# Banus/pano360

Hardware: AMD Instinct MI355X
Metric: blended megapixels/sec (multiband) (higher is better)
Workload: dtype f32; 1 GPU; cfg3: 32 synthetic 3840x2160 frames per image set, spherical warp + multiband blend L=5, native resolution (MAX_RESOLUTION uncapped); frames=32

## Files before the change

### include/pano360.h

```cpp
#ifndef PANO360_H
#define PANO360_H

#include <stddef.h>
#include <stdint.h>

#ifdef __cplusplus
extern "C" {
#endif

#define PANO_OK 0
#define PANO_EINVAL (-1)
#define PANO_EHIP (-2)
#define PANO_ELIMIT (-3)
#define PANO_ESOLVE (-4)

#define PANO_MAX_TAPS 129
#define PANO_MAX_LEVELS 8
#define PANO_TAP_LEAD 7
#define PANO_TAP_PAD 40
#ifndef PANO_INTERIOR_BLOCK
#define PANO_INTERIOR_BLOCK 4
#endif

typedef struct pano_patch {
// ... 38 lines not shown
    float angle;
    float response;
    int32_t octave;
    int32_t r, c;
} pano_sift_keypoint;


const char *pano_version(void);
const char *pano_last_error(void);
int pano_device_count(void);
int pano_pitch(int w);
int pano_interior_block(void);

typedef struct pano_ctx pano_ctx;
#define PANO_OPT_BLUR_KERNEL 0
#define PANO_OPT_OWN_PRUNE 1
#define PANO_OPT_BLUR_SEGMENTS 2
#define PANO_OPT_BLUR_LEAN 3
#define PANO_OPT_STITCH_STREAMS 4
#define PANO_OPT_STITCH_ASYNC 5
#define PANO_OPT_BLUR_SEG_LEN 6
#define PANO_OPT_SIFT_GRAPH 7
#define PANO_OPT_LEVEL_CLASSES 8
#define PANO_OPT_COUNT 9
#define PANO_BLUR_MFMA 0
#define PANO_BLUR_VALU 1
int pano_ctx_create(int device, void *stream, pano_ctx **out);
int pano_ctx_destroy(pano_ctx *ctx);
int pano_ctx_set_stream(pano_ctx *ctx, void *stream);
int pano_ctx_set_option(pano_ctx *ctx, int option, int value);
int pano_ctx_get_option(const pano_ctx *ctx, int option, int *value);

int pano_timing_enable(pano_ctx *ctx, int on);
int pano_kernel_count(void);
const char *pano_kernel_name(int kid);
int pano_timing_read(pano_ctx *ctx, int kid, double *total_ms, int *launches);

int pano_add_weights(pano_ctx *ctx, const uint8_t *frame, int h, int w,
                     const float *lut255, const double *hat_x, const double *hat_y,
                     float *rgba);

int pano_warp_spherical(pano_ctx *ctx, const uint8_t *frame, int sh, int sw,
                        const double *proj, const double *sin_t, const double *cos_t,
                        const double *tan_p, const float *lut255, const double *hat_x,
                        const double *hat_y, int gx0, int gy0, int pw, int ph,
                        float *planes, uint8_t *mask, float *map_x, float *map_y);

// ... 257 lines not shown
```

### pano360_amd/_lib.py

```python
import ctypes as C
import os
import subprocess

_HERE = os.path.dirname(os.path.abspath(__file__))
LIB_PATH = os.environ.get("PANO_LIB") or os.path.join(_HERE, "libpano360_hip.so")

MAX_TAPS = 129
MAX_LEVELS = 8
TAP_LEAD = 7
TAP_PAD = 40
OPT_BLUR_KERNEL, OPT_OWN_PRUNE, OPT_BLUR_SEGMENTS, OPT_BLUR_LEAN, OPT_STITCH_STREAMS = 0, 1, 2, 3, 4
OPT_STITCH_ASYNC = 5
OPT_BLUR_SEG_LEN = 6
OPT_SIFT_GRAPH = 7
OPT_LEVEL_CLASSES = 8
BLUR_MFMA, BLUR_VALU = 0, 1


class PanoError(RuntimeError):
    """A C-ABI call returned a negative status."""


class Patch(C.Structure):
    _fields_ = [("planes", C.c_void_p), ("mask", C.c_void_p),
                ("blurred", C.c_void_p), ("scratch", C.c_void_p),
                ("y0", C.c_int32), ("x0", C.c_int32), ("h", C.c_int32), ("w", C.c_int32),
                ("vy0", C.c_int32), ("vx0", C.c_int32), ("vh", C.c_int32), ("vw", C.c_int32),
                ("ay0", C.c_int32), ("ax0", C.c_int32), ("ah", C.c_int32), ("aw", C.c_int32),
                ("vpitch", C.c_int32), ("apitch", C.c_int32),
                ("index", C.c_int32), ("tiles_off", C.c_int32)]


class Layout(C.Structure):
    _fields_ = [("planes_floats", C.c_int64), ("blurred_floats", C.c_int64),
                ("scratch_floats", C.c_int64), ("n_records", C.c_int32), ("n_tiles", C.c_int32),
                ("max_vw", C.c_int32), ("max_vh", C.c_int32), ("max_aw", C.c_int32),
                ("max_ah", C.c_int32), ("missing", C.c_int32)]

# ... 205 lines not shown
```

### pano360_amd/csrc/api.hip

```cpp
#include <stdarg.h>
#include <stdio.h>
#include <stdlib.h>
#include <string.h>

#include <vector>

#include "common.h"
#include "layout.h"

static thread_local char g_error[512] = "";

void pano_set_error(const char *fmt, ...) {
    va_list ap;
    va_start(ap, fmt);
    vsnprintf(g_error, sizeof(g_error), fmt, ap);
    va_end(ap);
}

extern "C" const char *pano_version(void) { return "pano360_hip 0.1 (gfx950)"; }

extern "C" const char *pano_last_error(void) { return g_error; }

extern "C" int pano_device_count(void) {
    int n = 0;
// ... 8 lines not shown

extern "C" int pano_interior_block(void) { return PANO_INTERIOR_BLOCK; }

extern "C" int pano_ctx_create(int device, void *stream, pano_ctx **out) {
    PANO_REQUIRE(out, "pano_ctx_create: null output");
    *out = nullptr;
    PANO_REQUIRE(device >= 0 && device < pano_device_count(), "pano_ctx_create: no device %d",
                 device);
    PANO_HIP(hipSetDevice(device));
    if (int rc = pano_blur_mfma_opt_in()) return rc;
    if (int rc = pano_blur_valu_opt_in()) return rc;
    pano_ctx *ctx = new pano_ctx();
    ctx->device = device;
    ctx->stream = (hipStream_t)stream;
    ctx->opt[PANO_OPT_BLUR_KERNEL] = PANO_BLUR_MFMA;
    ctx->opt[PANO_OPT_OWN_PRUNE] = 1;
    ctx->opt[PANO_OPT_BLUR_SEGMENTS] = 1;
    ctx->opt[PANO_OPT_BLUR_LEAN] = 1;
    ctx->opt[PANO_OPT_STITCH_STREAMS] = 1;
    ctx->opt[PANO_OPT_STITCH_ASYNC] = 0;
    ctx->opt[PANO_OPT_BLUR_SEG_LEN] = 0;
    ctx->opt[PANO_OPT_SIFT_GRAPH] = 1;
    ctx->opt[PANO_OPT_LEVEL_CLASSES] = 0;
    *out = ctx;
    return PANO_OK;
}

int pano_ctx_enter(pano_ctx *ctx) {
    if (!ctx->in_stitch) ctx->geom_valid = false;
    PANO_HIP(hipSetDevice(ctx->device));
    return PANO_OK;
}

static void timing_clear(pano_ctx *ctx) {
    for (int k = 0; k < PK_COUNT; ++k) {
        for (hipEvent_t e : ctx->t_begin[k]) (void)hipEventDestroy(e);
        for (hipEvent_t e : ctx->t_end[k]) (void)hipEventDestroy(e);
        ctx->t_begin[k].clear();
        ctx->t_end[k].clear();
    }
}

static void tap_set_free(PanoTapSet &ts) {
    if (ts.taps) (void)hipFree(ts.taps);
    if (ts.tables) (void)hipFree(ts.tables);
    if (ts.ready) (void)hipEventDestroy(ts.ready);
// ... 151 lines not shown
    return PANO_OK;
}

int pano_ctx_tap_set_built(pano_ctx *ctx, PanoTapSet *set) {
    PANO_HIP(hipEventRecord(set->ready, ctx->stream));
    set->built_on = ctx->stream;
    return PANO_OK;
}

static const char *const g_kernel_names[] = {
    "add_weights_kernel", "warp_spherical_kernel", "ownership_kernel", "blur_rows_kernel",
    "blur_cols_kernel",   "multiband_compose_kernel", "linear_blend_kernel",
    "no_blend_kernel",    "crop_heights_kernel", "crop_rows_kernel", "pyr_down_kernel",
    "ownership_cameras_kernel", "owned_boxes_kernel", "warp_windows_kernel",
    "blend_cameras_kernel", "owned_spans_kernel",
    "block_owner_kernel", "tile_flags_kernel", "overlap_stats_kernel",
    "blur_mfma_kernel", "sift_extrema_kernel", "sift_orient_kernel", "sift_describe_kernel",
    "scale_step_kernel", "knn2_kernel", "blur_lean_kernel", "blur_lean5_kernel",
    "ransac_score_kernel", "ransac_finish_kernel", "match_pack_kernel",
    "ba_residual_kernel", "ba_pair_kernel", "ba_assemble_kernel",
    "jpeg_destuff_kernel", "jpeg_scan_kernel", "jpeg_intervals_kernel", "jpeg_huff_sync_kernel",
    "jpeg_huff_write_kernel", "jpeg_dc_kernel", "jpeg_idct_kernel", "jpeg_pixels_kernel",
    "jpeg_enc_blocks_kernel", "jpeg_enc_count_kernel", "jpeg_enc_scan_kernel", "jpeg_enc_emit_kernel",
    "jpeg_enc_stuff_kernel"};
static_assert(sizeof(g_kernel_names) / sizeof(g_kernel_names[0]) == PK_COUNT,
              "one name per PanoKernelId, in enum order");

void pano_timing_edge(pano_ctx *ctx, int kid, hipStream_t stream, bool begin) {
    hipEvent_t ev;
    if (hipEventCreate(&ev) != hipSuccess) return;
    (void)hipEventRecord(ev, stream);
    (begin ? ctx->t_begin : ctx->t_end)[kid].push_back(ev);
}

extern "C" int pano_timing_enable(pano_ctx *ctx, int on) {
    PANO_REQUIRE(ctx, "pano_timing_enable: null context");
    timing_clear(ctx);
    ctx->timing_on = on != 0;
    return PANO_OK;
}

extern "C" int pano_kernel_count(void) { return PK_COUNT; }

extern "C" const char *pano_kernel_name(int kid) {
    return kid >= 0 && kid < PK_COUNT ? g_kernel_names[kid] : "";
}

// ... 83 lines not shown
```

### pano360_amd/csrc/blend.hip

```cpp
#include <stdlib.h>

#include "geom.h"

__global__ __launch_bounds__(256) void ownership_kernel(
    const pano_patch *__restrict__ patches, int n, int H, int W,
    int16_t *__restrict__ owner, uint8_t *__restrict__ valid) {
    const int x = blockIdx.x * 64 + threadIdx.x, y = blockIdx.y * 4 + threadIdx.y;
    if (x >= W || y >= H) return;
    float best = 0.0f;
    int who = -1;
    bool any = false;
    for (int i = 0; i < n; ++i) {
        const pano_patch p = patches[i];
        const int px = x - p.x0, py = y - p.y0;
        if ((unsigned)px >= (unsigned)p.w || (unsigned)py >= (unsigned)p.h) continue;
        const float a = p.planes[3 * (size_t)p.vh * p.vpitch + (size_t)py * p.vpitch + px];
        if (a > best) {
            best = a;
            who = i;
        }
        any |= p.mask[(size_t)py * p.w + px] == 0;
    }
    owner[(size_t)y * W + x] = (int16_t)who;
    valid[(size_t)y * W + x] = any ? 1 : 0;
// ... 643 lines not shown
enum { LUT_LDS = 0, LUT_GLOBAL = 1 };

template <int LUT>
__device__ __forceinline__ void shade_interior(const pano_camera *cam, const float *__restrict__ table,
                                               const InteriorArgs &ia, int x, int y, int W,
                                               uint8_t *__restrict__ mosaic,
                                               float *__restrict__ mosaic_f32) {
    if (!cam->frame) return;
    const int sw = cam->sw, sh = cam->sh;
    float fx, fy;
    map_pixel(cam->proj, table_f64(ia.sin_t, x), table_f64(ia.cos_t, x), table_f64(ia.tan_p, y), sw, sh, fx, fy);
    Taps tp = tap_base(fx, fy);
    TapBytes tb;
    if (__ballot(!taps_interior(tp, sw, sh)) == 0ull) {
        tb = load_taps_interior(cam->frame, sw, tp);
    } else {
        tp.x1 = min(tp.x1, sw - 1);
        tp.y1 = min(tp.y1, sh - 1);
        tb = load_taps(cam->frame, sw, tp);
    }
    const size_t g = ((size_t)y * W + x) * 3;
#pragma unroll
    for (int c = 0; c < 3; ++c) {
        float v = lerp4(lut_at(table, tb.v[0][c]), lut_at(table, tb.v[1][c]),
                        lut_at(table, tb.v[2][c]), lut_at(table, tb.v[3][c]), tp);
        v = v < 0.0f ? 0.0f : (v > 1.0f ? 1.0f : v);
        if (mosaic_f32) mosaic_f32[g + c] = v;
        mosaic[g + c] = (uint8_t)(int)(255.0f * v);
    }
}

template <int LUT>
__device__ __forceinline__ void shade_interior_of(int own, const float *__restrict__ table, int stride,
                                                  const InteriorArgs &ia, int x, int y, int W,
                                                  uint8_t *__restrict__ mosaic,
                                                  float *__restrict__ mosaic_f32) {
    const int own_u = __builtin_amdgcn_readfirstlane(own);
    if (__ballot(own != own_u) == 0)
        shade_interior<LUT>(ia.cams + own_u, table + (size_t)own_u * stride, ia, x, y, W, mosaic, mosaic_f32);
    else
        shade_interior<LUT>(ia.cams + own, table + (size_t)own * stride, ia, x, y, W, mosaic, mosaic_f32);
}

#define COMPOSE_MASKS 4
template <int L, bool PERCAM, bool CLS>
__global__ __launch_bounds__(256) void multiband_compose_kernel(
    const pano_patch *__restrict__ patches, int n, int H, int W, int xs0, int xs1,
    const int16_t *__restrict__ owner, const uint8_t *__restrict__ valid,
    uint8_t *__restrict__ mosaic, float *__restrict__ mosaic_f32, InteriorArgs ia) {
    __shared__ float s_lut[256];
    if (ia.interior && !PERCAM) {
        s_lut[threadIdx.y * 64 + threadIdx.x] = ia.lut[threadIdx.y * 64 + threadIdx.x];
        __syncthreads();
    }
    const int x = xs0 + blockIdx.x * 64 + threadIdx.x, y = blockIdx.y * 4 + threadIdx.y;
    const bool inside = x < xs1 && y < H;
    const bool is_interior = inside && ia.interior && ia.interior[(size_t)(y / IB) * ia.W8 + x / IB];
    unsigned long long cand[COMPOSE_MASKS] = {};
    const bool masked = n <= 64 * COMPOSE_MASKS && __ballot(inside && !is_interior) != 0;
    if (masked) {
        const int wx0 = xs0 + blockIdx.x * 64, wx1 = min(wx0 + 64, xs1);
#pragma unroll
        for (int m = 0; m < COMPOSE_MASKS; ++m) {
            const int i = 64 * m + (int)threadIdx.x;
            bool hit = false;
            if (i < n) {
                const pano_patch *q = patches + i;
                const int ax = q->x0 + q->ax0, ay = q->y0 + q->ay0;
                hit = ax < wx1 && ax + q->aw > wx0 && ay <= y && y < ay + q->ah;
            }
            cand[m] = __ballot(hit);
        }
    }
    if (!inside) return;
    if (is_interior) {
        const int own = owner[(size_t)y * W + x];
        if (PERCAM)
            shade_interior_of<LUT_GLOBAL>(own, ia.lut, 256, ia, x, y, W, mosaic, mosaic_f32);
        else
            shade_interior_of<LUT_LDS>(own, s_lut, 0, ia, x, y, W, mosaic, mosaic_f32);
        return;
    }
    float layer[L][3], wsum[L];
#pragma unroll
    for (int k = 0; k < L; ++k) layer[k][0] = layer[k][1] = layer[k][2] = wsum[k] = 0.0f;
    const int j = CLS && L > 1 ? (int)ia.classes[(size_t)(y / IB) * ia.W8 + x / IB] : 0;
    const int own_px = CLS && j > 0 ? (int)owner[(size_t)y * W + x] : -1;
    float base[3] = {0.0f, 0.0f, 0.0f};

    int m = 0;
    unsigned long long bits = masked ? cand[0] : 0ull;
    for (int i = 0;; ++i) {
        if (masked) {
            while (bits == 0ull && ++m < COMPOSE_MASKS) bits = cand[m];
            if (bits == 0ull) break;
            i = 64 * m + __ffsll((long long)bits) - 1;
            bits &= bits - 1ull;
        } else if (i >= n) {
// ... 353 lines not shown
extern "C" int pano_interior_map(pano_ctx *ctx, const int16_t *owner, int H, int W, int xs0,
                                 int xs1, int radius, int16_t *block_owner, uint8_t *interior) {
    PANO_ENTER(ctx, "pano_interior_map");
    return interior_map_launch(ctx, owner, H, W, xs0, xs1, &radius, 1, block_owner, interior, nullptr,
                               "pano_interior_map");
}

extern "C" int pano_interior_classes(pano_ctx *ctx, const int16_t *owner, int H, int W, int xs0,
                                     int xs1, const int *radii, int n_radii, int16_t *block_owner,
                                     uint8_t *interior, uint8_t *classes) {
    PANO_ENTER(ctx, "pano_interior_classes");
    PANO_REQUIRE(classes, "pano_interior_classes: null pointer");
    return interior_map_launch(ctx, owner, H, W, xs0, xs1, radii, n_radii, block_owner, interior,
                               classes, "pano_interior_classes");
}

extern "C" int pano_multiband_compose(pano_ctx *ctx, const pano_patch *patches, int n, int H,
                                      int W, int xs0, int xs1, int n_levels, const int16_t *owner,
                                      const uint8_t *valid, const uint8_t *interior,
                                      const uint8_t *classes, const pano_camera *cams,
                                      const double *sin_t,
                                      const double *cos_t, const double *tan_p, const float *lut,
                                      int lut_stride, uint8_t *mosaic, float *mosaic_f32) {
    PANO_ENTER(ctx, "pano_multiband_compose");
    if (int rc = check_table(patches, n, H, W, "pano_multiband_compose")) return rc;
    PANO_REQUIRE(H > 0 && W > 0, "pano_multiband_compose: bad mosaic shape %dx%d", H, W);
    PANO_REQUIRE(owner && mosaic && valid, "pano_multiband_compose: null pointer");
    PANO_REQUIRE(n_levels >= 1 && n_levels <= PANO_MAX_LEVELS,
                 "pano_multiband_compose: n_levels %d outside [1, %d]", n_levels, PANO_MAX_LEVELS);
    PANO_REQUIRE(xs0 >= 0 && xs1 <= W && xs0 <= xs1,
                 "pano_multiband_compose: bad strip [%d, %d)", xs0, xs1);
    PANO_REQUIRE(!interior || (cams && sin_t && cos_t && tan_p && lut),
                 "pano_multiband_compose: the interior map needs cameras, tables and LUT");
    PANO_REQUIRE(lut_stride == 0 || lut_stride == 256,
                 "pano_multiband_compose: lut_stride %d (0 = shared table, 256 = per camera)",
                 lut_stride);
    if (xs0 == xs1) return PANO_OK;
    PANO_REQUIRE(!classes || interior, "pano_multiband_compose: level classes without the interior map");
    InteriorArgs ia = {interior, ceil_div(W, IB), cams, sin_t, cos_t, tan_p, lut,
                       ctx->opt[PANO_OPT_LEVEL_CLASSES] ? classes : nullptr};
    const bool percam = interior && lut_stride != 0;
    dim3 block(64, 4), grid(ceil_div(xs1 - xs0, 64), ceil_div(H, 4));
    hipStream_t s = (hipStream_t)stream;
#define COMPOSE_AS(L, PC, CL)                                                            \
    PANO_TIMED(PK_COMPOSE, s,                                                           \
               hipLaunchKernelGGL((multiband_compose_kernel<L, PC, CL>), grid, block, 0, s, \
                                  patches, n, H, W, xs0, xs1, owner, valid, mosaic,     \
                                  mosaic_f32, ia))
#define COMPOSE(L)                                                                      \
    case L:                                                                             \
        if (ia.classes && L > 1) {                                                      \
            if (percam) COMPOSE_AS(L, true, true); else COMPOSE_AS(L, false, true);     \
        } else {                                                                        \
            if (percam) COMPOSE_AS(L, true, false); else COMPOSE_AS(L, false, false);   \
        }                                                                               \
        break;
    switch (n_levels) {
        COMPOSE(1) COMPOSE(2) COMPOSE(3) COMPOSE(4) COMPOSE(5) COMPOSE(6) COMPOSE(7) COMPOSE(8)
    }
#undef COMPOSE_AS
#undef COMPOSE
    PANO_LAUNCH_CHECK("multiband_compose_kernel");
    return PANO_OK;
}

extern "C" int pano_linear_blend(pano_ctx *ctx, const pano_patch *patches, int n, int H, int W,
                                 uint8_t *mosaic) {
    PANO_ENTER(ctx, "pano_linear_blend");
    if (int rc = check_table(patches, n, H, W, "pano_linear_blend")) return rc;
    PANO_REQUIRE(mosaic, "pano_linear_blend: null output");
    MOSAIC_GRID;
    PANO_TIMED(PK_LINEAR, (hipStream_t)stream,
               hipLaunchKernelGGL(linear_blend_kernel, grid, block, 0, (hipStream_t)stream,
                                  patches, n, H, W, mosaic));
    PANO_LAUNCH_CHECK("linear_blend_kernel");
    return PANO_OK;
}

extern "C" int pano_no_blend(pano_ctx *ctx, const pano_patch *patches, int n, int H, int W,
                             uint8_t *mosaic) {
    PANO_ENTER(ctx, "pano_no_blend");
    if (int rc = check_table(patches, n, H, W, "pano_no_blend")) return rc;
    PANO_REQUIRE(mosaic, "pano_no_blend: null output");
// ... 8 lines not shown
```

### pano360_amd/csrc/common.h

```cpp
#pragma once
#include <hip/hip_runtime.h>
#include <stdint.h>

#include <vector>

#include "../../include/pano360.h"

void pano_set_error(const char *fmt, ...);

#define PANO_REQUIRE(cond, ...)          \
    do {                                 \
        if (!(cond)) {                   \
            pano_set_error(__VA_ARGS__); \
            return PANO_EINVAL;          \
        }                                \
    } while (0)

#define PANO_HIP(call)                                                         \
    do {                                                                       \
        hipError_t e_ = (call);                                                \
        if (e_ != hipSuccess) {                                                \
            pano_set_error("%s failed: %s", #call, hipGetErrorString(e_));     \
            return PANO_EHIP;                                                  \
        }                                                                      \
// ... 36 lines not shown
    PK_SCALE_STEP,
    PK_KNN2,
    PK_BLUR_LEAN,
    PK_BLUR_LEAN5,
    PK_RANSAC_SCORE,
    PK_RANSAC_FINISH,
    PK_MATCH_PACK,
    PK_BA_RESIDUAL,
    PK_BA_PAIRS,
    PK_BA_ASSEMBLE,
    PK_JPEG_DESTUFF,
    PK_JPEG_SCAN,
    PK_JPEG_INTERVALS,
    PK_JPEG_HUFF_SYNC,
    PK_JPEG_HUFF_WRITE,
    PK_JPEG_DC,
    PK_JPEG_IDCT,
    PK_JPEG_PIXELS,
    PK_JPEG_ENC_BLOCKS,
    PK_JPEG_ENC_COUNT,
    PK_JPEG_ENC_SCAN,
    PK_JPEG_ENC_EMIT,
    PK_JPEG_ENC_STUFF,
    PK_COUNT
};
struct PanoTapSet {
    uint64_t key;
    int n, ntaps[PANO_MAX_LEVELS];
    float *taps;
    unsigned char *tables;
    uint64_t used;
    float *host;
    size_t floats;
    hipEvent_t ready;
    hipStream_t built_on;
};

struct LayoutSummary;
struct PanoSiftGraph {
    uint64_t key;
    hipGraphExec_t exec;
    int seen;
    uint64_t used;
};

#define GEOM_BUFS 11
// ... 32 lines not shown
    bool geom_valid, in_stitch;
    const void *geom_bufs[GEOM_BUFS];
    int lay_count[2];
    uint32_t *sift_raw;
    size_t sift_raw_cap;
    bool sift_capturing;
    std::vector<PanoSiftGraph> sift_graphs;
    uint8_t *enc_dev, *enc_out, *enc_host;
    size_t enc_dev_cap, enc_out_cap, enc_host_cap;
    uint8_t *poisson_dev, *poisson_host;
    size_t poisson_cap;
    uint8_t *seam_dev, *seam_host;
};

int pano_ctx_enter(pano_ctx *ctx);
void pano_sift_graphs_free(pano_ctx *ctx);
int pano_sift_raw_reserve(pano_ctx *ctx, int rows, int cols);
int pano_zero_i32(hipStream_t s, int *p, int n);
int pano_ctx_side_stream(pano_ctx *ctx);
int pano_ctx_tap_set(pano_ctx *ctx, const float *taps, const int *ntaps, int n, size_t table_bytes,
                     PanoTapSet **out, bool *fresh);
int pano_ctx_tap_set_built(pano_ctx *ctx, PanoTapSet *set);

#define PANO_ENTER(ctx, who)                                       \
    PANO_REQUIRE((ctx) != nullptr, "%s: null context", who);       \
    if (int rc_ = pano_ctx_enter(ctx)) return rc_;                 \
    void *const stream = (void *)(ctx)->stream;                    \
    (void)stream

#define PANO_ENTER_READONLY(ctx, who)                              \
    const bool geom_keep_ = (ctx) != nullptr && (ctx)->geom_valid; \
    PANO_ENTER(ctx, who);                                          \
    (ctx)->geom_valid = geom_keep_

void pano_timing_edge(pano_ctx *ctx, int kid, hipStream_t stream, bool begin);

#define PANO_TIMED(kid, stream, ...)                                        \
    do {                                                                    \
        if (ctx->timing_on) pano_timing_edge(ctx, kid, stream, true);       \
        __VA_ARGS__;                                                        \
        if (ctx->timing_on) pano_timing_edge(ctx, kid, stream, false);      \
    } while (0)

static inline int pano_pitch_of(int w) { return (w + 3) & ~3; }

int pano_launch_blur_mfma(pano_ctx *ctx, const pano_patch *table, int n, int max_aw, int max_ah,
// ... 42 lines not shown
```

### pano360_amd/csrc/geom.h

```cpp
#pragma once
#include "common.h"

struct Taps {
    int x0, x1, y0, y1;
    float w00, w01, w10, w11;
};

__device__ __forceinline__ Taps tap_base(float px, float py) {
    int sx = cv_round(px * 32.0f), sy = cv_round(py * 32.0f);
    int fx = sx & 31, fy = sy & 31;
    Taps t;
    t.x0 = sat16(sx >> 5);
    t.y0 = sat16(sy >> 5);
    t.x1 = t.x0 + 1;
    t.y1 = t.y0 + 1;
    float ax = (float)fx * (1.0f / 32.0f), ay = (float)fy * (1.0f / 32.0f);
    t.w00 = (1.0f - ay) * (1.0f - ax);
    t.w01 = (1.0f - ay) * ax;
    t.w10 = ay * (1.0f - ax);
    t.w11 = ay * ax;
    return t;
}

__device__ __forceinline__ void reflect_taps(Taps &t, int sw, int sh) {
// ... 7 lines not shown
    Taps t = tap_base(px, py);
    reflect_taps(t, sw, sh);
    return t;
}

__device__ __forceinline__ bool taps_interior(const Taps &t, int sw, int sh) {
    return (unsigned)t.x0 < (unsigned)(sw - 1) && (unsigned)t.y0 < (unsigned)(sh - 1);
}

__device__ __forceinline__ Taps make_taps_unmasked(float px, float py, int sw, int sh) {
    Taps t = tap_base(px, py);
    t.x1 = min(t.x1, sw - 1);
    t.y1 = min(t.y1, sh - 1);
    return t;
}

__device__ __forceinline__ float lerp4(float v00, float v01, float v10, float v11,
                                       const Taps &t) {
    float a = v00 * t.w00;
    a = a + v01 * t.w01;
    a = a + v10 * t.w10;
    a = a + v11 * t.w11;
    return a;
}

struct TapBytes {
    uint32_t v[4][3];
};
typedef uint32_t u32_any __attribute__((aligned(1)));
typedef uint16_t u16_any __attribute__((aligned(1)));
typedef const __attribute__((address_space(1))) uint8_t *frame_ptr;
typedef const __attribute__((address_space(1))) u32_any *frame_ptr32;
typedef const __attribute__((address_space(1))) u16_any *frame_ptr16;

#define PANO_BYTE_X4(B)                                                                        \
    __device__ __forceinline__ uint32_t byte##B##_x4(uint32_t x) {                             \
        uint32_t r;                                                                            \
        asm("v_lshlrev_b32_sdwa %0, %1, %2 dst_sel:DWORD dst_unused:UNUSED_PAD "               \
            "src0_sel:DWORD src1_sel:BYTE_" #B                                                 \
            : "=v"(r)                                                                          \
            : "v"(2u), "v"(x));                                                                \
        return r;                                                                              \
    }
PANO_BYTE_X4(0)
PANO_BYTE_X4(1)
PANO_BYTE_X4(2)
// ... 84 lines not shown
```

### pano360_amd/csrc/stitch.hip

```cpp
#include <string.h>

#include "common.h"
#include "layout.h"


#define LAY_THREADS 512
__global__ __launch_bounds__(LAY_THREADS) void layout_windows_kernel(
    const int32_t *__restrict__ regions, const int32_t *__restrict__ rects,
    const uint8_t *__restrict__ have, int n, int max_spans, int radius, int xs0, int xs1,
    int n_blur, int grid32, float *planes, float *blurred, float *scratch, long cap_planes,
    long cap_blurred, long cap_scratch, int cap_tiles, int want_tiles, int b_nr, int b_vw,
    int b_vh, int b_aw, int b_ah, pano_patch *__restrict__ table,
    LayoutSummary *__restrict__ summary, LayoutSummary expect, int check_expect,
    int *__restrict__ sticky) {
    __shared__ long s_planes[LAY_THREADS], s_blurred[LAY_THREADS], s_scratch[LAY_THREADS];
    __shared__ int s_tiles[LAY_THREADS], s_slot[LAY_THREADS];
    __shared__ long s_run[4];
    __shared__ int s_count, s_max[4], s_missing, s_bad;
    const int tid = threadIdx.x, stride = 5 + 2 * max_spans;
    if (tid == 0) {
        s_run[0] = s_run[1] = s_run[2] = s_run[3] = 0;
        s_count = s_missing = s_bad = 0;
        s_max[0] = s_max[1] = s_max[2] = s_max[3] = 0;
    }
// ... 204 lines not shown
    }
    a->used_need = 0;
    if (kept) {
        a->used_need = need_choice == 1;
        two_streams = false;
    } else if (interior && tile_grid == 32 && nr && a->tile_flags && a->need) {
        bool on = need_choice == 1;
        if (need_choice < 0) {
            double sum = 0.0;
            for (int k = 0; k < nr; ++k) sum += a->records_host[k].aw;
            on = sum / nr >= 768.0;
        }
        if (on) {
            if (two_streams) {
                PANO_HIP(hipEventRecord(ctx->ev_join, ctx->side));
                PANO_HIP(hipStreamWaitEvent(s, ctx->ev_join, 0));
            }
            if (int rc = pano_blur_tiles(ctx, a->table, nr, lay.max_aw, lay.max_ah, a->W, a->radius,
                                         a->interior, a->tile_flags, a->need))
                return rc;
            a->used_need = 1;
        }
    }
    const bool fork2 = two_streams && interior && n_blur && nr &&
                       !a->used_need && tile_grid == 32 && a->tile_flags;
    if (fork2) {
        if (device_table) {
            PANO_HIP(hipEventRecord(ctx->ev_upload, s));
        }
        PANO_HIP(hipStreamWaitEvent(ctx->side, ctx->ev_upload, 0));
        ON_SIDE(ctx, pano_multiband_blur_prepare(ctx, a->table, nr, lay.max_aw, lay.max_ah, a->W,
                                                 a->interior, a->tile_flags));
        PANO_HIP(hipEventRecord(ctx->ev_join, ctx->side));
    } else if (two_streams && interior) {
        PANO_HIP(hipEventRecord(ctx->ev_join, ctx->side));
    }
    if (int rc = pano_warp_windows(ctx, a->cams, a->table, nr, lay.max_vw, lay.max_vh, a->sin_t,
                                   a->cos_t, a->tan_p, a->lut, a->lut_stride,
                                   a->used_need ? a->need : nullptr))
        return rc;
    if (two_streams && interior) PANO_HIP(hipStreamWaitEvent(s, ctx->ev_join, 0));
    if (kept && use_blur) {
        ctx->prepared_table = a->table;
        ctx->prepared_n = nr;
    }
    if (n_blur)
        if (int rc = pano_multiband_blur(ctx, a->table, nr, lay.max_aw, lay.max_vh, lay.max_ah,
                                         a->owner, a->W, a->taps, (const int *)a->ntaps, n_blur,
                                         interior ? a->interior : nullptr,
                                         interior ? a->tile_flags : nullptr))
            return rc;
    return pano_multiband_compose(ctx, a->table, nr, a->H, a->W, a->xs0, a->xs1, a->n_levels,
                                  a->owner, a->valid, interior ? a->interior : nullptr,
                                  interior && stitch_has_classes(ctx, a, n_blur) ? a->classes : nullptr,
                                  interior ? a->cams : nullptr, interior ? a->sin_t : nullptr,
                                  interior ? a->cos_t : nullptr, interior ? a->tan_p : nullptr,
                                  a->lut, a->lut_stride, a->mosaic, a->mosaic_f32);
}

static void geometry_buffers(const pano_stitch_args *a, const void *out[GEOM_BUFS]) {
    const void *v[GEOM_BUFS] = {a->owner, a->valid, a->table, a->interior, a->tile_flags, a->need,
                                a->planes, a->blurred, a->scratch, a->sin_t, a->classes};
    for (int k = 0; k < GEOM_BUFS; ++k) out[k] = v[k];
}
static void geometry_left(pano_ctx *ctx, const pano_stitch_args *a) {
    geometry_buffers(a, ctx->geom_bufs);
    ctx->geom_valid = true;
}

namespace {
struct StitchScope {
    pano_ctx *ctx;
    explicit StitchScope(pano_ctx *c) : ctx(c) { ctx->in_stitch = true; }
    ~StitchScope() { ctx->in_stitch = false; }
};
}

extern "C" int pano_stitch_multiband(pano_ctx *ctx, pano_stitch_args *a, int resume) {
    const bool geom_was_valid = ctx && ctx->geom_valid;
    PANO_ENTER(ctx, "pano_stitch_multiband");
// ... 225 lines not shown
```

### pano360_amd/csrc/warp.hip

```cpp
#include "geom.h"

struct ProjK {
    double p[9];
};

template <bool FULL>
__global__ __launch_bounds__(256) void warp_spherical_kernel(
    const uint8_t *__restrict__ frame, int sh, int sw, ProjK K,
    const double *__restrict__ sin_t, const double *__restrict__ cos_t,
    const double *__restrict__ tan_p, const float *__restrict__ lut255,
    const double *__restrict__ hat_x, const double *__restrict__ hat_y,
    int gx0, int gy0, int pw, int ph, int pitch, float *__restrict__ planes,
    uint8_t *__restrict__ mask, float *__restrict__ map_x,
    float *__restrict__ map_y) {
    __shared__ float s_lut[256];
    s_lut[threadIdx.y * 64 + threadIdx.x] = lut255[threadIdx.y * 64 + threadIdx.x];
    __syncthreads();

    const int x = blockIdx.x * 64 + threadIdx.x;
    const int y = blockIdx.y * 4 + threadIdx.y;
    if (x >= pw || y >= ph) return;

    float px, py;
    const bool m = map_pixel(K.p, sin_t[gx0 + x], cos_t[gx0 + x], tan_p[gy0 + y], sw, sh,
// ... 2 lines not shown
    const uint8_t *r0 = frame + (size_t)tp.y0 * sw * 3;
    const uint8_t *r1 = frame + (size_t)tp.y1 * sw * 3;
    const uint8_t *p00 = r0 + tp.x0 * 3, *p01 = r0 + tp.x1 * 3;
    const uint8_t *p10 = r1 + tp.x0 * 3, *p11 = r1 + tp.x1 * 3;
    const size_t plane = (size_t)ph * pitch;
    const size_t o = (size_t)y * pitch + x;
#pragma unroll
    for (int k = 0; k < 3; ++k)
        planes[k * plane + o] =
            lerp4(s_lut[p00[k]], s_lut[p01[k]], s_lut[p10[k]], s_lut[p11[k]], tp);
    if (FULL) {
        float a = alpha_at(hat_x, hat_y, tp);
        a = a * (m ? 0.0f : 1.0f);
        planes[3 * plane + o] = a;
        mask[(size_t)y * pw + x] = m ? 1 : 0;
        if (map_x) {
            map_x[(size_t)y * pw + x] = px;
            map_y[(size_t)y * pw + x] = py;
        }
    }
}

#define WARP_ROWS 4
__global__ __launch_bounds__(256) void warp_windows_kernel(
    const pano_camera *__restrict__ cams, const pano_patch *__restrict__ patches,
    const double *__restrict__ sin_t, const double *__restrict__ cos_t,
    const double *__restrict__ tan_p, const float *__restrict__ lut, int lut_stride,
    const uint8_t *__restrict__ need) {
    __shared__ float s_lut[256];
    const pano_patch p = patches[blockIdx.z];
    constexpr int BH = 4 * WARP_ROWS;
    if ((int)blockIdx.x * 64 >= p.vw || (int)blockIdx.y * BH >= p.vh) return;
    if (need) {
        const int ntx = ((p.ax0 + p.aw - 1) >> 5) - (p.ax0 >> 5) + 1;
        const int nty = ((p.ay0 + p.ah - 1) >> 5) - (p.ay0 >> 5) + 1;
        const int px0 = p.vx0 + (int)blockIdx.x * 64, py0 = p.vy0 + (int)blockIdx.y * BH;
        const int ty0 = min(max((py0 >> 5) - (p.ay0 >> 5), 0), nty - 1);
        const int ty1 = min(max(((py0 + BH - 1) >> 5) - (p.ay0 >> 5), 0), nty - 1);
        const int tx0 = min(max((px0 >> 5) - (p.ax0 >> 5), 0), ntx - 1);
        const int tx1 = min(max(((px0 + 63) >> 5) - (p.ax0 >> 5), 0), ntx - 1);
        bool any = false;
        for (int ty = ty0; ty <= ty1; ++ty)
            for (int tx = tx0; tx <= tx1; ++tx) any |= need[p.tiles_off + ty * ntx + tx] != 0;
        if (!any) return;
    }
    s_lut[threadIdx.y * 64 + threadIdx.x] =
        lut[(size_t)p.index * lut_stride + threadIdx.y * 64 + threadIdx.x];
    __syncthreads();

    const int x = blockIdx.x * 64 + threadIdx.x;
    const int y0 = blockIdx.y * BH + threadIdx.y;
    if (x >= p.vw || y0 >= p.vh) return;
    const pano_camera *cam = cams + p.index;
    const int sw = cam->sw, sh = cam->sh;
    const int gx = p.x0 + p.vx0 + x;
    const double s = table_f64(sin_t, gx), c = table_f64(cos_t, gx);
    double t[WARP_ROWS];
#pragma unroll
    for (int j = 0; j < WARP_ROWS; ++j)
        t[j] = table_f64(tan_p, p.y0 + p.vy0 + min(y0 + 4 * j, p.vh - 1));
    Taps tp[WARP_ROWS];
    TapBytes tb[WARP_ROWS];
    bool inner = true;
#pragma unroll
    for (int j = 0; j < WARP_ROWS; ++j) {
        float px, py;
        map_pixel(cam->proj, s, c, t[j], sw, sh, px, py);
        tp[j] = tap_base(px, py);
        inner &= taps_interior(tp[j], sw, sh);
    }
    if (__ballot(!inner) == 0ull) {
#pragma unroll
        for (int j = 0; j < WARP_ROWS; ++j) tb[j] = load_taps_interior(cam->frame, sw, tp[j]);
    } else {
#pragma unroll
        for (int j = 0; j < WARP_ROWS; ++j) {
            reflect_taps(tp[j], sw, sh);
            tb[j] = load_taps(cam->frame, sw, tp[j]);
        }
    }
    typedef __attribute__((address_space(1))) float *plane_ptr;
    typedef __attribute__((address_space(1))) char *byte_ptr;
    const size_t plane = (size_t)p.vh * p.vpitch;
    const byte_ptr out[3] = {(byte_ptr)p.planes, (byte_ptr)(p.planes + plane),
                             (byte_ptr)(p.planes + 2 * plane)};
#pragma unroll
    for (int j = 0; j < WARP_ROWS; ++j) {
        const int y = y0 + 4 * j;
        if (y >= p.vh) break;
        const uint32_t o = ((uint32_t)y * (uint32_t)p.vpitch + (uint32_t)x) * 4u;
#pragma unroll
        for (int k = 0; k < 3; ++k) {
            *(plane_ptr)(out[k] + o) = lerp4(lut_at(s_lut, tb[j].v[0][k]), lut_at(s_lut, tb[j].v[1][k]),
                                             lut_at(s_lut, tb[j].v[2][k]), lut_at(s_lut, tb[j].v[3][k]), tp[j]);
        }
    }
}

__global__ __launch_bounds__(256) void add_weights_kernel(
    const uint8_t *__restrict__ frame, int h, int w,
    const float *__restrict__ lut255, const double *__restrict__ hat_x,
    const double *__restrict__ hat_y, float4 *__restrict__ rgba) {
    const int x = blockIdx.x * 64 + threadIdx.x;
    const int y = blockIdx.y * 4 + threadIdx.y;
    if (x >= w || y >= h) return;
    const uint8_t *s = frame + ((size_t)y * w + x) * 3;
    float4 v;
    v.x = lut255[s[0]];
    v.y = lut255[s[1]];
    v.z = lut255[s[2]];
    v.w = (float)(hat_y[y] * hat_x[x]);
    rgba[(size_t)y * w + x] = v;
}

extern "C" int pano_add_weights(pano_ctx *ctx, const uint8_t *frame, int h, int w,
                                const float *lut255, const double *hat_x, const double *hat_y,
                                float *rgba) {
// ... 31 lines not shown
    for (int i = 0; i < 9; ++i) K.p[i] = proj[i];
    dim3 block(64, 4), grid(ceil_div(pw, 64), ceil_div(ph, 4));
    PANO_TIMED(PK_WARP, (hipStream_t)stream,
               hipLaunchKernelGGL(warp_spherical_kernel<true>, grid, block, 0,
                                  (hipStream_t)stream, frame, sh, sw, K, sin_t, cos_t, tan_p,
                                  lut255, hat_x, hat_y, gx0, gy0, pw, ph, pano_pitch_of(pw),
                                  planes, mask, map_x, map_y));
    PANO_LAUNCH_CHECK("warp_spherical_kernel");
    return PANO_OK;
}

extern "C" int pano_warp_windows(pano_ctx *ctx, const pano_camera *cams, const pano_patch *patches,
                                 int n, int max_vw, int max_vh, const double *sin_t,
                                 const double *cos_t, const double *tan_p, const float *lut,
                                 int lut_stride, const uint8_t *need) {
    PANO_ENTER(ctx, "pano_warp_windows");
    PANO_REQUIRE(cams && patches && sin_t && cos_t && tan_p && lut && lut_stride >= 0,
                 "pano_warp_windows: null pointer");
    PANO_REQUIRE(n >= 0 && n <= 65535 && max_vw >= 0 && max_vh >= 0,
                 "pano_warp_windows: bad argument");
    if (n == 0 || max_vw == 0 || max_vh == 0) return PANO_OK;
    dim3 block(64, 4), grid(ceil_div(max_vw, 64), ceil_div(max_vh, 4 * WARP_ROWS), n);
    PANO_TIMED(PK_WARP_WINDOWS, (hipStream_t)stream,
               hipLaunchKernelGGL(warp_windows_kernel, grid, block, 0, (hipStream_t)stream,
                                  cams, patches, sin_t, cos_t, tan_p, lut, lut_stride, need));
    PANO_LAUNCH_CHECK("warp_windows_kernel");
    return PANO_OK;
}
```

Baseline: 209,900 MP/s.

## Fuse interior mosaic shading into the window warp kernel

When the interior map is available and level classes are off, the window warp kernel also writes the final 8-bit (and optional f32) mosaic pixels for interior blocks owned by the current camera. It packs RGB bytes across the wavefront with shuffles so rows are stored as aligned dwords. The compose kernel then runs an unshaded variant that skips interior pixels, so the separate per-pixel re-projection and bilinear resampling in compose goes away. The cost is extra owner and interior-map reads in warp, masked byte stores, and a new stream join before the warp, which serializes the side stream earlier.

```diff
diff --git a/include/pano360.h b/include/pano360.h
--- a/include/pano360.h
+++ b/include/pano360.h
@@ -84,7 +84,8 @@
 #define PANO_OPT_BLUR_SEG_LEN 6
 #define PANO_OPT_SIFT_GRAPH 7
 #define PANO_OPT_LEVEL_CLASSES 8
-#define PANO_OPT_COUNT 9
+#define PANO_OPT_WARP_INTERIOR 9
+#define PANO_OPT_COUNT 10
 #define PANO_BLUR_MFMA 0
 #define PANO_BLUR_VALU 1
 int pano_ctx_create(int device, void *stream, pano_ctx **out);
diff --git a/pano360_amd/_lib.py b/pano360_amd/_lib.py
--- a/pano360_amd/_lib.py
+++ b/pano360_amd/_lib.py
@@ -14,6 +14,7 @@
 OPT_BLUR_SEG_LEN = 6
 OPT_SIFT_GRAPH = 7
 OPT_LEVEL_CLASSES = 8
+OPT_WARP_INTERIOR = 9
 BLUR_MFMA, BLUR_VALU = 0, 1
 
 
diff --git a/pano360_amd/csrc/api.hip b/pano360_amd/csrc/api.hip
--- a/pano360_amd/csrc/api.hip
+++ b/pano360_amd/csrc/api.hip
@@ -54,6 +54,7 @@
     ctx->opt[PANO_OPT_BLUR_SEG_LEN] = 0;
     ctx->opt[PANO_OPT_SIFT_GRAPH] = 1;
     ctx->opt[PANO_OPT_LEVEL_CLASSES] = 0;
+    ctx->opt[PANO_OPT_WARP_INTERIOR] = 1;
     *out = ctx;
     return PANO_OK;
 }
@@ -251,7 +252,7 @@
     "jpeg_destuff_kernel", "jpeg_scan_kernel", "jpeg_intervals_kernel", "jpeg_huff_sync_kernel",
     "jpeg_huff_write_kernel", "jpeg_dc_kernel", "jpeg_idct_kernel", "jpeg_pixels_kernel",
     "jpeg_enc_blocks_kernel", "jpeg_enc_count_kernel", "jpeg_enc_scan_kernel", "jpeg_enc_emit_kernel",
-    "jpeg_enc_stuff_kernel"};
+    "jpeg_enc_stuff_kernel", "warp_windows_mosaic_kernel", "multiband_compose_seams_kernel"};
 static_assert(sizeof(g_kernel_names) / sizeof(g_kernel_names[0]) == PK_COUNT,
               "one name per PanoKernelId, in enum order");
 
diff --git a/pano360_amd/csrc/blend.hip b/pano360_amd/csrc/blend.hip
--- a/pano360_amd/csrc/blend.hip
+++ b/pano360_amd/csrc/blend.hip
@@ -689,11 +689,11 @@
     const size_t g = ((size_t)y * W + x) * 3;
 #pragma unroll
     for (int c = 0; c < 3; ++c) {
-        float v = lerp4(lut_at(table, tb.v[0][c]), lut_at(table, tb.v[1][c]),
-                        lut_at(table, tb.v[2][c]), lut_at(table, tb.v[3][c]), tp);
-        v = v < 0.0f ? 0.0f : (v > 1.0f ? 1.0f : v);
+        float v;
+        const uint8_t q = interior_channel(lerp4(lut_at(table, tb.v[0][c]), lut_at(table, tb.v[1][c]),
+                                                 lut_at(table, tb.v[2][c]), lut_at(table, tb.v[3][c]), tp), v);
         if (mosaic_f32) mosaic_f32[g + c] = v;
-        mosaic[g + c] = (uint8_t)(int)(255.0f * v);
+        mosaic[g + c] = q;
     }
 }
 
@@ -710,13 +710,13 @@
 }
 
 #define COMPOSE_MASKS 4
-template <int L, bool PERCAM, bool CLS>
+template <int L, bool PERCAM, bool CLS, bool SHADE>
 __global__ __launch_bounds__(256) void multiband_compose_kernel(
     const pano_patch *__restrict__ patches, int n, int H, int W, int xs0, int xs1,
     const int16_t *__restrict__ owner, const uint8_t *__restrict__ valid,
     uint8_t *__restrict__ mosaic, float *__restrict__ mosaic_f32, InteriorArgs ia) {
     __shared__ float s_lut[256];
-    if (ia.interior && !PERCAM) {
+    if (SHADE && ia.interior && !PERCAM) {
         s_lut[threadIdx.y * 64 + threadIdx.x] = ia.lut[threadIdx.y * 64 + threadIdx.x];
         __syncthreads();
     }
@@ -741,6 +741,7 @@
     }
     if (!inside) return;
     if (is_interior) {
+        if (!SHADE) return;
         const int own = owner[(size_t)y * W + x];
         if (PERCAM)
             shade_interior_of<LUT_GLOBAL>(own, ia.lut, 256, ia, x, y, W, mosaic, mosaic_f32);
@@ -1140,6 +1141,17 @@
                                       const double *sin_t,
                                       const double *cos_t, const double *tan_p, const float *lut,
                                       int lut_stride, uint8_t *mosaic, float *mosaic_f32) {
+    return pano_multiband_compose_as(ctx, patches, n, H, W, xs0, xs1, n_levels, owner, valid, interior,
+                                     classes, cams, sin_t, cos_t, tan_p, lut, lut_stride, mosaic,
+                                     mosaic_f32, true);
+}
+
+int pano_multiband_compose_as(pano_ctx *ctx, const pano_patch *patches, int n, int H, int W, int xs0,
+                              int xs1, int n_levels, const int16_t *owner, const uint8_t *valid,
+                              const uint8_t *interior, const uint8_t *classes,
+                              const pano_camera *cams, const double *sin_t, const double *cos_t,
+                              const double *tan_p, const float *lut, int lut_stride, uint8_t *mosaic,
+                              float *mosaic_f32, bool shade) {
     PANO_ENTER(ctx, "pano_multiband_compose");
     if (int rc = check_table(patches, n, H, W, "pano_multiband_compose")) return rc;
     PANO_REQUIRE(H > 0 && W > 0, "pano_multiband_compose: bad mosaic shape %dx%d", H, W);
@@ -1158,16 +1170,26 @@
     InteriorArgs ia = {interior, ceil_div(W, IB), cams, sin_t, cos_t, tan_p, lut,
                        ctx->opt[PANO_OPT_LEVEL_CLASSES] ? classes : nullptr};
     const bool percam = interior && lut_stride != 0;
+    PANO_REQUIRE(shade || (interior && !ia.classes),
+                 "pano_multiband_compose: the unshaded collapse needs the interior map and no level classes");
     dim3 block(64, 4), grid(ceil_div(xs1 - xs0, 64), ceil_div(H, 4));
     hipStream_t s = (hipStream_t)stream;
 #define COMPOSE_AS(L, PC, CL)                                                            \
     PANO_TIMED(PK_COMPOSE, s,                                                           \
-               hipLaunchKernelGGL((multiband_compose_kernel<L, PC, CL>), grid, block, 0, s, \
+               hipLaunchKernelGGL((multiband_compose_kernel<L, PC, CL, true>), grid, block, 0, s, \
                                   patches, n, H, W, xs0, xs1, owner, valid, mosaic,     \
                                   mosaic_f32, ia))
+#define COMPOSE_SEAMS(L)                                                                \
+    PANO_TIMED(PK_COMPOSE, s,                                                           \
+               PANO_TIMED(PK_COMPOSE_SEAMS, s,                                          \
+                          hipLaunchKernelGGL((multiband_compose_kernel<L, false, false, false>), grid, \
+                                             block, 0, s, patches, n, H, W, xs0, xs1, owner, valid, \
+                                             mosaic, mosaic_f32, ia)))
 #define COMPOSE(L)                                                                      \
     case L:                                                                             \
-        if (ia.classes && L > 1) {                                                      \
+        if (!shade) {                                                                   \
+            COMPOSE_SEAMS(L);                                                           \
+        } else if (ia.classes && L > 1) {                                               \
             if (percam) COMPOSE_AS(L, true, true); else COMPOSE_AS(L, false, true);     \
         } else {                                                                        \
             if (percam) COMPOSE_AS(L, true, false); else COMPOSE_AS(L, false, false);   \
@@ -1177,6 +1199,7 @@
         COMPOSE(1) COMPOSE(2) COMPOSE(3) COMPOSE(4) COMPOSE(5) COMPOSE(6) COMPOSE(7) COMPOSE(8)
     }
 #undef COMPOSE_AS
+#undef COMPOSE_SEAMS
 #undef COMPOSE
     PANO_LAUNCH_CHECK("multiband_compose_kernel");
     return PANO_OK;
diff --git a/pano360_amd/csrc/common.h b/pano360_amd/csrc/common.h
--- a/pano360_amd/csrc/common.h
+++ b/pano360_amd/csrc/common.h
@@ -82,6 +82,8 @@
     PK_JPEG_ENC_SCAN,
     PK_JPEG_ENC_EMIT,
     PK_JPEG_ENC_STUFF,
+    PK_WARP_WINDOWS_MOSAIC,
+    PK_COMPOSE_SEAMS,
     PK_COUNT
 };
 struct PanoTapSet {
@@ -160,6 +162,24 @@
                      PanoTapSet **out, bool *fresh);
 int pano_ctx_tap_set_built(pano_ctx *ctx, PanoTapSet *set);
 
+struct WarpMosaic {
+    const int16_t *owner;
+    const uint8_t *interior;
+    uint8_t *mosaic;
+    float *mosaic_f32;
+    int H, W, W8, xs0, xs1;
+};
+int pano_warp_windows_mosaic(pano_ctx *ctx, const pano_camera *cams, const pano_patch *patches, int n,
+                             int max_vw, int max_vh, const double *sin_t, const double *cos_t,
+                             const double *tan_p, const float *lut, int lut_stride,
+                             const WarpMosaic &wm);
+int pano_multiband_compose_as(pano_ctx *ctx, const pano_patch *patches, int n, int H, int W, int xs0,
+                              int xs1, int n_levels, const int16_t *owner, const uint8_t *valid,
+                              const uint8_t *interior, const uint8_t *classes,
+                              const pano_camera *cams, const double *sin_t, const double *cos_t,
+                              const double *tan_p, const float *lut, int lut_stride, uint8_t *mosaic,
+                              float *mosaic_f32, bool shade);
+
 #define PANO_ENTER(ctx, who)                                       \
     PANO_REQUIRE((ctx) != nullptr, "%s: null context", who);       \
     if (int rc_ = pano_ctx_enter(ctx)) return rc_;                 \
diff --git a/pano360_amd/csrc/geom.h b/pano360_amd/csrc/geom.h
--- a/pano360_amd/csrc/geom.h
+++ b/pano360_amd/csrc/geom.h
@@ -53,6 +53,32 @@
     a = a + v10 * t.w10;
     a = a + v11 * t.w11;
     return a;
+}
+
+__device__ __forceinline__ uint8_t interior_channel(float v, float &clipped) {
+    v = v < 0.0f ? 0.0f : (v > 1.0f ? 1.0f : v);
+    clipped = v;
+    return (uint8_t)(int)(255.0f * v);
+}
+
+__device__ __forceinline__ void store_rgb_row(uint8_t *__restrict__ row, uint32_t pix) {
+    const int a = (int)((uintptr_t)row & 3u);
+    const int r0 = 4 * (int)threadIdx.x - a;
+    const int s0 = (r0 + 3) / 3 - 1;
+    const int c = r0 - 3 * s0;
+    const uint32_t p0 = __shfl(pix, s0 & 63, 64), p1 = __shfl(pix, (s0 + 1) & 63, 64);
+    const bool w0 = (unsigned)s0 < 64u && (p0 >> 24) != 0;
+    const bool w1 = (unsigned)(s0 + 1) < 64u && (p1 >> 24) != 0;
+    const uint64_t both = (uint64_t)(p0 & 0xffffffu) | ((uint64_t)(p1 & 0xffffffu) << 24);
+    const uint32_t dw = (uint32_t)(both >> (8 * c));
+    uint8_t *dst = row + r0;
+    if (w0 && w1) {
+        *(uint32_t *)dst = dw;
+    } else if (w0 || w1) {
+#pragma unroll
+        for (int i = 0; i < 4; ++i)
+            if (c + i < 3 ? w0 : w1) dst[i] = (uint8_t)(dw >> (8 * i));
+    }
 }
 
 struct TapBytes {
diff --git a/pano360_amd/csrc/stitch.hip b/pano360_amd/csrc/stitch.hip
--- a/pano360_amd/csrc/stitch.hip
+++ b/pano360_amd/csrc/stitch.hip
@@ -250,6 +250,13 @@
             a->used_need = 1;
         }
     }
+    const bool warp_interior = interior && tile_grid == 32 && n_blur > 0 && nr > 0 && !a->used_need &&
+                               ctx->opt[PANO_OPT_WARP_INTERIOR] != 0 &&
+                               !stitch_has_classes(ctx, a, n_blur);
+    if (warp_interior && two_streams) {
+        PANO_HIP(hipEventRecord(ctx->ev_join, ctx->side));
+        PANO_HIP(hipStreamWaitEvent(s, ctx->ev_join, 0));
+    }
     const bool fork2 = two_streams && interior && n_blur && nr &&
                        !a->used_need && tile_grid == 32 && a->tile_flags;
     if (fork2) {
@@ -263,9 +270,15 @@
     } else if (two_streams && interior) {
         PANO_HIP(hipEventRecord(ctx->ev_join, ctx->side));
     }
-    if (int rc = pano_warp_windows(ctx, a->cams, a->table, nr, lay.max_vw, lay.max_vh, a->sin_t,
-                                   a->cos_t, a->tan_p, a->lut, a->lut_stride,
-                                   a->used_need ? a->need : nullptr))
+    if (warp_interior) {
+        const WarpMosaic wm = {a->owner, a->interior, a->mosaic, a->mosaic_f32, a->H, a->W,
+                               ceil_div(a->W, PANO_INTERIOR_BLOCK), a->xs0, a->xs1};
+        if (int rc = pano_warp_windows_mosaic(ctx, a->cams, a->table, nr, lay.max_vw, lay.max_vh,
+                                              a->sin_t, a->cos_t, a->tan_p, a->lut, a->lut_stride, wm))
+            return rc;
+    } else if (int rc = pano_warp_windows(ctx, a->cams, a->table, nr, lay.max_vw, lay.max_vh, a->sin_t,
+                                          a->cos_t, a->tan_p, a->lut, a->lut_stride,
+                                          a->used_need ? a->need : nullptr))
         return rc;
     if (two_streams && interior) PANO_HIP(hipStreamWaitEvent(s, ctx->ev_join, 0));
     if (kept && use_blur) {
@@ -278,12 +291,12 @@
                                          interior ? a->interior : nullptr,
                                          interior ? a->tile_flags : nullptr))
             return rc;
-    return pano_multiband_compose(ctx, a->table, nr, a->H, a->W, a->xs0, a->xs1, a->n_levels,
-                                  a->owner, a->valid, interior ? a->interior : nullptr,
-                                  interior && stitch_has_classes(ctx, a, n_blur) ? a->classes : nullptr,
-                                  interior ? a->cams : nullptr, interior ? a->sin_t : nullptr,
-                                  interior ? a->cos_t : nullptr, interior ? a->tan_p : nullptr,
-                                  a->lut, a->lut_stride, a->mosaic, a->mosaic_f32);
+    return pano_multiband_compose_as(ctx, a->table, nr, a->H, a->W, a->xs0, a->xs1, a->n_levels,
+                                     a->owner, a->valid, interior ? a->interior : nullptr,
+                                     interior && stitch_has_classes(ctx, a, n_blur) ? a->classes : nullptr,
+                                     interior ? a->cams : nullptr, interior ? a->sin_t : nullptr,
+                                     interior ? a->cos_t : nullptr, interior ? a->tan_p : nullptr,
+                                     a->lut, a->lut_stride, a->mosaic, a->mosaic_f32, !warp_interior);
 }
 
 static void geometry_buffers(const pano_stitch_args *a, const void *out[GEOM_BUFS]) {
diff --git a/pano360_amd/csrc/warp.hip b/pano360_amd/csrc/warp.hip
--- a/pano360_amd/csrc/warp.hip
+++ b/pano360_amd/csrc/warp.hip
@@ -48,11 +48,12 @@
 }
 
 #define WARP_ROWS 4
+template <bool MOSAIC>
 __global__ __launch_bounds__(256) void warp_windows_kernel(
     const pano_camera *__restrict__ cams, const pano_patch *__restrict__ patches,
     const double *__restrict__ sin_t, const double *__restrict__ cos_t,
     const double *__restrict__ tan_p, const float *__restrict__ lut, int lut_stride,
-    const uint8_t *__restrict__ need) {
+    const uint8_t *__restrict__ need, WarpMosaic wm) {
     __shared__ float s_lut[256];
     const pano_patch p = patches[blockIdx.z];
     constexpr int BH = 4 * WARP_ROWS;
@@ -74,9 +75,11 @@
         lut[(size_t)p.index * lut_stride + threadIdx.y * 64 + threadIdx.x];
     __syncthreads();
 
-    const int x = blockIdx.x * 64 + threadIdx.x;
+    const int xr = blockIdx.x * 64 + threadIdx.x;
     const int y0 = blockIdx.y * BH + threadIdx.y;
-    if (x >= p.vw || y0 >= p.vh) return;
+    const bool live = xr < p.vw;
+    if ((!MOSAIC && !live) || y0 >= p.vh) return;
+    const int x = MOSAIC ? min(xr, p.vw - 1) : xr;
     const pano_camera *cam = cams + p.index;
     const int sw = cam->sw, sh = cam->sh;
     const int gx = p.x0 + p.vx0 + x;
@@ -115,10 +118,28 @@
         const int y = y0 + 4 * j;
         if (y >= p.vh) break;
         const uint32_t o = ((uint32_t)y * (uint32_t)p.vpitch + (uint32_t)x) * 4u;
+        float v[3];
 #pragma unroll
         for (int k = 0; k < 3; ++k) {
-            *(plane_ptr)(out[k] + o) = lerp4(lut_at(s_lut, tb[j].v[0][k]), lut_at(s_lut, tb[j].v[1][k]),
-                                             lut_at(s_lut, tb[j].v[2][k]), lut_at(s_lut, tb[j].v[3][k]), tp[j]);
+            v[k] = lerp4(lut_at(s_lut, tb[j].v[0][k]), lut_at(s_lut, tb[j].v[1][k]),
+                         lut_at(s_lut, tb[j].v[2][k]), lut_at(s_lut, tb[j].v[3][k]), tp[j]);
+            if (!MOSAIC || live) *(plane_ptr)(out[k] + o) = v[k];
+        }
+        if (MOSAIC) {
+            const int gy = p.y0 + p.vy0 + y;
+            bool mine = live && gx >= wm.xs0 && gx < wm.xs1 && (unsigned)gy < (unsigned)wm.H;
+            if (mine) mine = wm.interior[(size_t)(gy / PANO_INTERIOR_BLOCK) * wm.W8 + gx / PANO_INTERIOR_BLOCK] != 0;
+            if (mine) mine = wm.owner[(size_t)gy * wm.W + gx] == p.index;
+            const size_t g = ((size_t)gy * wm.W + gx) * 3;
+            uint32_t pix = mine ? 1u << 24 : 0u;
+#pragma unroll
+            for (int k = 0; k < 3; ++k) {
+                float clipped;
+                pix |= (uint32_t)interior_channel(v[k], clipped) << (8 * k);
+                if (mine && wm.mosaic_f32) wm.mosaic_f32[g + k] = clipped;
+            }
+            const long long row = ((long long)gy * wm.W + (p.x0 + p.vx0 + (int)blockIdx.x * 64)) * 3;
+            store_rgb_row(wm.mosaic + row, pix);
         }
     }
 }
@@ -196,8 +217,31 @@
     if (n == 0 || max_vw == 0 || max_vh == 0) return PANO_OK;
     dim3 block(64, 4), grid(ceil_div(max_vw, 64), ceil_div(max_vh, 4 * WARP_ROWS), n);
     PANO_TIMED(PK_WARP_WINDOWS, (hipStream_t)stream,
-               hipLaunchKernelGGL(warp_windows_kernel, grid, block, 0, (hipStream_t)stream,
-                                  cams, patches, sin_t, cos_t, tan_p, lut, lut_stride, need));
+               hipLaunchKernelGGL(warp_windows_kernel<false>, grid, block, 0, (hipStream_t)stream,
+                                  cams, patches, sin_t, cos_t, tan_p, lut, lut_stride, need,
+                                  WarpMosaic{}));
     PANO_LAUNCH_CHECK("warp_windows_kernel");
     return PANO_OK;
 }
+
+int pano_warp_windows_mosaic(pano_ctx *ctx, const pano_camera *cams, const pano_patch *patches, int n,
+                             int max_vw, int max_vh, const double *sin_t, const double *cos_t,
+                             const double *tan_p, const float *lut, int lut_stride,
+                             const WarpMosaic &wm) {
+    PANO_ENTER(ctx, "pano_warp_windows_mosaic");
+    PANO_REQUIRE(cams && patches && sin_t && cos_t && tan_p && lut && lut_stride >= 0 && wm.owner &&
+                     wm.interior && wm.mosaic,
+                 "pano_warp_windows_mosaic: null pointer");
+    PANO_REQUIRE(n >= 0 && n <= 65535 && max_vw >= 0 && max_vh >= 0 && wm.H > 0 && wm.W > 0 &&
+                     wm.xs0 >= 0 && wm.xs0 <= wm.xs1 && wm.xs1 <= wm.W && wm.W8 == ceil_div(wm.W, PANO_INTERIOR_BLOCK),
+                 "pano_warp_windows_mosaic: bad argument");
+    if (n == 0 || max_vw == 0 || max_vh == 0) return PANO_OK;
+    dim3 block(64, 4), grid(ceil_div(max_vw, 64), ceil_div(max_vh, 4 * WARP_ROWS), n);
+    PANO_TIMED(PK_WARP_WINDOWS, (hipStream_t)stream,
+               PANO_TIMED(PK_WARP_WINDOWS_MOSAIC, (hipStream_t)stream,
+                          hipLaunchKernelGGL(warp_windows_kernel<true>, grid, block, 0,
+                                             (hipStream_t)stream, cams, patches, sin_t, cos_t, tan_p,
+                                             lut, lut_stride, nullptr, wm)));
+    PANO_LAUNCH_CHECK("warp_windows_kernel");
+    return PANO_OK;
+}
```

After: 216,800 MP/s (median of 6 runs). +3.3%, better.
